# khanhha/temporal_inverse_kinematics

Hardware: AMD Instinct MI355X
Metric: IK frames/sec (COCO-17->SMPLx pose) (higher is better)
Workload: dtype f32 via bf16x3 (x = 3 bf16 planes, 6 MFMA products, fp32 accumulate; fp32 exponent range); 1 GPU; ST-GCN IK forward, batch=1024x64-frame x COCO-17 windows per GPU -> (B,4,66) SMPL-X pose; global_batch=1024, window_frames=64, out_frames=4, parallelism=single

## Files before the change

### temporal_inverse_kinematics_amd/csrc/xblock.hip

```cpp
#include <algorithm>
#include <type_traits>

#include "xgemm_dev.h"
#include "xblock.h"
#include "common.h"

namespace tik {

namespace xb {
constexpr int V = 17, C = 64, F = 10, FIN = F + 2;
constexpr int ROWB = 3 * C * 2;
constexpr int ZROWS = FIN * V;
constexpr int ZBYTES = (ZROWS + 1) * ROWB;
constexpr int XUNITS = ZROWS * 24, XINST = (XUNITS + 63) / 64;
constexpr int XBYTES = XINST * 1024;
constexpr int B2BYTES = V * C * 4;
constexpr int SMEM1 = ZBYTES + XBYTES + B2BYTES;
constexpr int F0 = 14, FIN0 = F0 + 2;
constexpr int ZBYTES0 = (FIN0 * V + 1) * ROWB;
constexpr int KPBYTES0 = FIN0 * V * 4 * 4;
constexpr int UBYTES0 = FIN0 * V * 16;
constexpr int SMEM0 = ZBYTES0 + KPBYTES0 + UBYTES0;
static_assert(SMEM1 <= 163840 && SMEM0 <= 163840, "LDS");
}

__device__ __forceinline__ int xb_unit(int R, int plane, int u) { return R * xb::ROWB + plane * 128 + ((u ^ (R & 7)) << 4); }
__device__ __forceinline__ int xb_xunit(int R, int j, int plane, int u) { return R * xb::ROWB + plane * 128 + ((u ^ ((R + j) & 7)) << 4); }

template <bool RAW>
__global__ __launch_bounds__(512, 1) void xblock_kernel(XBlkArgs a) {
    using namespace xb;
    constexpr int F = RAW ? F0 : xb::F, FIN = F + 2, ZROWS = FIN * V, ZR = ZROWS, ZBYTES = (ZROWS + 1) * ROWB;
    constexpr int KPBYTES = FIN * V * 4 * 4;
    constexpr int TPX = F * V, TBLK = (TPX + 15) / 16;
    static_assert(FIN <= 16, "one frame per lane of a 16-lane group");
    __shared__ __attribute__((aligned(16))) unsigned char smem[RAW ? SMEM0 : SMEM1];
    unsigned char* const zimg = smem;
    unsigned char* const ximg = smem + ZBYTES;
    float* const b2s = reinterpret_cast<float*>(smem + ZBYTES + XBYTES);

    int tid = threadIdx.x, lane = tid & 63;
    const int wave = __builtin_amdgcn_readfirstlane(tid >> 6);
    int g = lane >> 4;
    const int cg = wave & 3, ph = wave >> 2;
    const int QO = a.nframes, T = a.T;
    const int ntiles = (QO + F - 1) / F;
    int t_begin, t_end;
    {
        const int nwg = gridDim.x, bid = blockIdx.x;
        const int per = nwg >> 3, rem = nwg & 7, x = bid & 7, k = bid >> 3;
        const int s = x < rem ? x * (per + 1) + k : rem * (per + 1) + (x - rem) * per + k;
        t_begin = (int)((long long)s * ntiles / nwg);
        t_end = (int)((long long)(s + 1) * ntiles / nwg);
    }
    if (t_begin >= t_end) return;

    xbf16x8 wt[3][2][3];
    auto load_wt = [&]() __attribute__((always_inline)) {
        const unsigned short* wp = a.wtp;
        asm volatile("" : "+s"(wp));
#pragma unroll
        for (int k = 0; k < 3; ++k)
#pragma unroll
            for (int kb = 0; kb < 2; ++kb)
#pragma unroll
                for (int p = 0; p < 3; ++p)
                    wt[k][kb][p] = *reinterpret_cast<const xbf16x8*>(wp + ((((size_t)cg * 6 + k * 2 + kb) * 3 + p) * 64 + lane) * 8);
    };
    xbf16x8 wg[RAW ? 1 : 2][3];
    if constexpr (!RAW) {
#pragma unroll
        for (int kb = 0; kb < 2; ++kb)
#pragma unroll
            for (int p = 0; p < 3; ++p)
                wg[kb][p] = *reinterpret_cast<const xbf16x8*>(a.wgp + ((((size_t)cg * 2 + kb) * 3 + p) * 64 + lane) * 8);
    }
    float amv[5];
#pragma unroll
    for (int k = 0; k < 5; ++k) amv[k] = 64 * k + lane < V * V ? a.amix[64 * k + lane] : 0.f;
    int cho = 16 * cg + 4 * g;
    const f32x4 bv = *reinterpret_cast<const f32x4*>(a.bias + cho);
    float rw[4][4];
#pragma unroll
    for (int e = 0; e < 4; ++e)
#pragma unroll
        for (int c = 0; c < 4; ++c) rw[e][c] = RAW && c < a.c0 ? a.rw[(cho + e) * a.c0 + c] : 0.f;

    for (int i = tid; i < ROWB / 16; i += 512) *reinterpret_cast<f32x4*>(zimg + ZR * ROWB + 16 * i) = f32x4{0.f, 0.f, 0.f, 0.f};
    if constexpr (!RAW)
        for (int i = tid; i < V * C; i += 512) b2s[i] = a.bias2[i];

    const i32x4 rX = buf_rsrc(RAW ? nullptr : (const void*)a.xp3, RAW ? 0u : (unsigned)((long long)QO * V * ROWB));
    constexpr int NXI = (XINST + 7) / 8;
    unsigned xpre[NXI];
#pragma unroll
    for (int i = 0; i < NXI; ++i) {
        const int ins = wave + 8 * i;
        const int U = ins * 64 + lane;
        const int R = U / 24, k = U - R * 24, plane = k >> 3, up = k & 7;
        const int j = R / FIN, f = R - j * FIN;
        xpre[i] = U < XUNITS && ins < XINST ? (unsigned)((f * V + j) * ROWB + plane * 128 + ((up ^ ((R + j) & 7)) << 4)) | ((unsigned)f << 24)
                                            : 0x80000000u;
    }
    auto issue_x = [&](int tile) __attribute__((always_inline)) {
        const int q0 = tile * F;
#pragma unroll
        for (int i = 0; i < NXI; ++i) {
            const int ins = wave + 8 * i;
            if (ins >= XINST) break;
            const unsigned c = xpre[i];
            const int q = q0 - 1 + (int)((c >> 24) & 0x7F);
            const bool ok = !(c >> 31) && q >= 0 && q < QO;
            const unsigned off = ok ? (unsigned)((long long)(q0 - 1) * V * ROWB) + (c & 0xFFFFFFu) : DMA_OOB;
            tik_llvm_raw_buffer_load_lds(rX, (__attribute__((address_space(3))) unsigned*)(ximg + ins * 1024), 16, (int)off, 0, 0, 2);
        }
    };
    constexpr int KNE = RAW ? (FIN * V * 4 + 511) / 512 : 1;
    float kx[KNE], ksc[KNE], ksh[KNE];
    bool kok[KNE];
    auto load_kp = [&](int tile) __attribute__((always_inline)) {
#pragma unroll
        for (int jj = 0; jj < KNE; ++jj) {
            const int i = tid + 512 * jj, c = i & 3, p = i >> 2;
            const int v = p % V, fr = tile * F - 1 + p / V;
            kok[jj] = RAW && i < FIN * V * 4 && c < a.c0 && fr >= 0 && fr < QO;
            kx[jj] = kok[jj] ? a.xraw[((size_t)fr * V + v) * a.c0 + c] : 0.f;
        }
    };
    if constexpr (RAW) {
#pragma unroll
        for (int jj = 0; jj < KNE; ++jj) {
            const int i = tid + 512 * jj, c = i & 3, v = (i >> 2) % V;
            const bool ok = i < FIN * V * 4 && c < a.c0;
            ksc[jj] = ok ? a.bn_sc[v * a.c0 + c] : 0.f;
            ksh[jj] = ok ? a.bn_sh[v * a.c0 + c] : 0.f;
        }
        load_kp(t_begin);
    } else {
        asm volatile("s_waitcnt lgkmcnt(0)" ::: "memory");
        issue_x(t_begin);
    }

    constexpr int NB = (TBLK + 1) / 2;
    const int blk0 = ph * NB;
    const int nblk = ph == 0 ? NB : TBLK - NB;

#ifdef TIK_XTRACE
    const bool tr = a.trace != nullptr && (wave == 0 || wave == 4);
#else
    constexpr bool tr = false;
#endif
    unsigned long long ph_[8] = {0, 0, 0, 0, 0, 0, 0, 0}, tlast = 0;
    auto stamp = [&](int i) __attribute__((always_inline)) {
        if (tr) {
            const unsigned long long t = __builtin_amdgcn_s_memtime();
            if (i >= 0) ph_[i] += t - tlast;
            tlast = t;
        }
    };
    load_wt();
#pragma unroll
    for (int k = 0; k < 3; ++k)
#pragma unroll
        for (int kb = 0; kb < 2; ++kb)
#pragma unroll
            for (int p = 0; p < 3; ++p) asm volatile("" : "+v"(wt[k][kb][p]));
    for (int tile = t_begin; tile < t_end; ++tile) {
        const int q0 = tile * F;
        stamp(-1);
        asm volatile("" : "+v"(tid), "+v"(lane));
        g = lane >> 4;
        cho = 16 * cg + 4 * g;
        if constexpr (RAW) {
            float* kps = reinterpret_cast<float*>(ximg);
#pragma unroll
            for (int jj = 0; jj < KNE; ++jj) {
                const int i = tid + 512 * jj;
                if (i < FIN * V * 4) kps[i] = kok[jj] ? fmaf(kx[jj], ksc[jj], ksh[jj]) : 0.f;
            }
            __syncthreads();
            stamp(0);
            if (tile + 1 < t_end) load_kp(tile + 1);
            f32x4* const us = reinterpret_cast<f32x4*>(ximg + KPBYTES);
            {
                const int fl = lane;
                if (fl < FIN) {
#pragma unroll
                    for (int wj = 0; wj < V; ++wj)
                        if ((wj & 7) == wave) {
                            if (a.mix_sparse) us[fl * V + wj] = l0_mix_in<true>(kps + fl * V * 4, amv, wj);
                            else us[fl * V + wj] = l0_mix_in<false>(kps + fl * V * 4, amv, wj);
                        }
                }
            }
            __syncthreads();
            const int f = tid & 15, c4 = (tid >> 4) & 15, half = wave >> 2, co = 4 * c4;
            if (f < FIN) {
                float w[4][4];
#pragma unroll
                for (int e = 0; e < 4; ++e)
#pragma unroll
                    for (int c = 0; c < 4; ++c) w[e][c] = c < a.c0 ? a.wg0[(co + e) * a.ldwg0 + c] : 0.f;
                auto conv_half = [&](auto w0c, auto w1c) __attribute__((always_inline)) {
                    constexpr int W0 = decltype(w0c)::value, W1 = decltype(w1c)::value;
#pragma unroll
                    for (int wj = W0; wj < W1; ++wj) {
                        const f32x4 z = l0_conv_relu(us[f * V + wj], w, *reinterpret_cast<const f32x4*>(a.bias2 + wj * C + co));
                        xbf16x8 p0, p1, p2;
                        xsplit8(z, z, p0, p1, p2);
                        const int R = f * V + wj, u = co >> 3, o = (co & 7) * 2;
                        typedef __bf16 xbf16x4 __attribute__((ext_vector_type(4)));
                        *reinterpret_cast<xbf16x4*>(zimg + xb_unit(R, 0, u) + o) = xbf16x4{p0[0], p0[1], p0[2], p0[3]};
                        *reinterpret_cast<xbf16x4*>(zimg + xb_unit(R, 1, u) + o) = xbf16x4{p1[0], p1[1], p1[2], p1[3]};
                        *reinterpret_cast<xbf16x4*>(zimg + xb_unit(R, 2, u) + o) = xbf16x4{p2[0], p2[1], p2[2], p2[3]};
                    }
                };
                using I0 = std::integral_constant<int, 0>;
                using I9 = std::integral_constant<int, 9>;
                using I17 = std::integral_constant<int, 17>;
                if (half) conv_half(I9{}, I17{});
                else conv_half(I0{}, I9{});
            }
        } else {
            asm volatile("s_waitcnt vmcnt(0)" ::: "memory");
            __syncthreads();
            stamp(0);
            auto run_half = [&](auto jhc) __attribute__((always_inline)) {
                constexpr int JH = decltype(jhc)::value, J0 = JH ? 9 : 0, J1 = JH ? V : 9;
                f32x4 acc[V];
#pragma unroll
                for (int j = 0; j < V; ++j) acc[j] = f32x4{0.f, 0.f, 0.f, 0.f};
                const int fs = lane & 15, fr = fs < FIN ? fs : fs - FIN;
                constexpr int XPF = 2, S0 = 2 * J0, S1 = 2 * J1;
                xbf16x8 xb[XPF + 1][3];
                auto rd = [&](int s, xbf16x8 (&d)[3]) __attribute__((always_inline)) {
                    const int R = (s >> 1) * FIN + fr, kb = s & 1;
#pragma unroll
                    for (int p = 0; p < 3; ++p) d[p] = *reinterpret_cast<const xbf16x8*>(ximg + xb_xunit(R, s >> 1, p, 4 * kb + g));
                };
#pragma unroll
                for (int s = S0; s < S0 + XPF; ++s) rd(s, xb[(s - S0) % (XPF + 1)]);
#pragma unroll
                for (int s = S0; s < S1; ++s) {
                    const int j = s >> 1, kb = s & 1;
                    if (s + XPF < S1) rd(s + XPF, xb[(s + XPF - S0) % (XPF + 1)]);
                    __builtin_amdgcn_sched_barrier(0);
                    const xbf16x8(&x)[3] = xb[(s - S0) % (XPF + 1)];
                    acc[j] = __builtin_amdgcn_mfma_f32_16x16x32_bf16(wg[kb][0], x[2], acc[j], 0, 0, 0);
                    acc[j] = __builtin_amdgcn_mfma_f32_16x16x32_bf16(wg[kb][1], x[1], acc[j], 0, 0, 0);
                    acc[j] = __builtin_amdgcn_mfma_f32_16x16x32_bf16(wg[kb][2], x[0], acc[j], 0, 0, 0);
                    acc[j] = __builtin_amdgcn_mfma_f32_16x16x32_bf16(wg[kb][0], x[1], acc[j], 0, 0, 0);
                    acc[j] = __builtin_amdgcn_mfma_f32_16x16x32_bf16(wg[kb][1], x[0], acc[j], 0, 0, 0);
                    acc[j] = __builtin_amdgcn_mfma_f32_16x16x32_bf16(wg[kb][0], x[0], acc[j], 0, 0, 0);
                    __builtin_amdgcn_sched_barrier(0);
                }
                f32x4* xch = reinterpret_cast<f32x4*>(zimg);
#pragma unroll
                for (int j = J0; j < J1; ++j) xch[(j * 4 + cg) * 64 + lane] = acc[j];
                asm volatile("s_waitcnt lgkmcnt(0)" ::: "memory");
                __builtin_amdgcn_s_barrier();
#pragma unroll
                for (int j = 0; j < V; ++j)
                    if (j < J0 || j >= J1) acc[j] = xch[(j * 4 + cg) * 64 + lane];
                asm volatile("s_waitcnt lgkmcnt(0)" ::: "memory");
                __builtin_amdgcn_s_barrier();
                if (fs < FIN) {
                    auto mix_half = [&](auto sparse) __attribute__((always_inline)) {
                        constexpr bool SP = decltype(sparse)::value;
#pragma unroll
                        for (int w = J0; w < J1; ++w) {
                            f32x4 z = *reinterpret_cast<const f32x4*>(b2s + w * C + cho);
#pragma unroll
                            for (int v = 0; v < V; ++v)
                                if (!SP || ((coco_hop2_mask3(w) >> v) & 1u)) {
                                    const float av = __builtin_bit_cast(
                                        float, __builtin_amdgcn_readlane(__builtin_bit_cast(int, amv[(v * V + w) / 64]), (v * V + w) % 64));
                                    z += av * acc[v];
                                }
#pragma unroll
                            for (int e = 0; e < 4; ++e) z[e] = z[e] > 0.f ? z[e] : 0.f;
                            xbf16x8 p0, p1, p2;
                            xsplit8(z, z, p0, p1, p2);
                            const int R = fs * V + w, u = cho >> 3, o = (cho & 7) * 2;
                            typedef __bf16 xbf16x4 __attribute__((ext_vector_type(4)));
                            *reinterpret_cast<xbf16x4*>(zimg + xb_unit(R, 0, u) + o) = xbf16x4{p0[0], p0[1], p0[2], p0[3]};
                            *reinterpret_cast<xbf16x4*>(zimg + xb_unit(R, 1, u) + o) = xbf16x4{p1[0], p1[1], p1[2], p1[3]};
                            *reinterpret_cast<xbf16x4*>(zimg + xb_unit(R, 2, u) + o) = xbf16x4{p2[0], p2[1], p2[2], p2[3]};
                        }
                    };
                    if (a.mix_sparse) mix_half(std::true_type{});
                    else mix_half(std::false_type{});
                }
            };
            if (ph == 0) run_half(std::integral_constant<int, 0>{});
            else run_half(std::integral_constant<int, 1>{});
        }
        stamp(1);
        __syncthreads();
        stamp(2);

        f32x4 res[NB];
#pragma unroll
        for (int b = 0; b < NB; ++b) {
            const int p = (blk0 + b) * 16 + (lane & 15);
            const int fo = p / V, jt = p - fo * V;
            res[b] = f32x4{0.f, 0.f, 0.f, 0.f};
            if (b < nblk && p < TPX) {
                if constexpr (RAW) {
                    const float* xp = reinterpret_cast<const float*>(ximg) + ((fo + 1) * V + jt) * 4;
                    res[b] = f32x4{xp[0], xp[1], xp[2], xp[3]};
                } else {
                    const int R = jt * FIN + fo + 1, u = cho >> 3, o = (cho & 7) * 2;
                    typedef __bf16 xbf16x4 __attribute__((ext_vector_type(4)));
                    const xbf16x4 h0 = *reinterpret_cast<const xbf16x4*>(ximg + xb_xunit(R, jt, 0, u) + o);
                    const xbf16x4 h1 = *reinterpret_cast<const xbf16x4*>(ximg + xb_xunit(R, jt, 1, u) + o);
                    const xbf16x4 h2 = *reinterpret_cast<const xbf16x4*>(ximg + xb_xunit(R, jt, 2, u) + o);
#pragma unroll
                    for (int e = 0; e < 4; ++e) res[b][e] = ((float)h0[e] + (float)h1[e]) + (float)h2[e];
                }
            }
        }
        if constexpr (!RAW) {
            stamp(6);
            lds_barrier();
            if (tile + 1 < t_end) issue_x(tile + 1);
            stamp(7);
        }
        stamp(3);

        int rows[NB][3];
#pragma unroll
        for (int b = 0; b < NB; ++b) {
            const int p = (blk0 + b) * 16 + (lane & 15);
            const int fo = p / V, jt = p - fo * V;
            const int q = q0 + fo, tw = q % T;
#pragma unroll
            for (int k = 0; k < 3; ++k) {
                const bool ok = b < nblk && p < TPX && q < QO && tw + k - 1 >= 0 && tw + k - 1 < T;
                rows[b][k] = ok ? (fo + k) * V + jt : ZR;
            }
        }
        {
            constexpr int ZPF = 2, NS = 6 * NB;
            xbf16x8 zb[ZPF + 1][3];
            auto rdz = [&](int i, xbf16x8 (&d)[3]) __attribute__((always_inline)) {
                const int b = i / 6, s = i % 6, k = s % 3, kb = s / 3;
#pragma unroll
                for (int pl = 0; pl < 3; ++pl) d[pl] = *reinterpret_cast<const xbf16x8*>(zimg + xb_unit(rows[b][k], pl, 4 * kb + g));
            };
#pragma unroll
            for (int i = 0; i < ZPF; ++i) rdz(i, zb[i]);
            f32x4 acc = f32x4{0.f, 0.f, 0.f, 0.f};
#pragma unroll
            for (int i = 0; i < NS; ++i) {
                const int b = i / 6, s = i % 6;
                if (b >= nblk) break;
                if (i + ZPF < NS) rdz(i + ZPF, zb[(i + ZPF) % (ZPF + 1)]);
                __builtin_amdgcn_sched_barrier(0);
                const xbf16x8(&z)[3] = zb[i % (ZPF + 1)];
                const xbf16x8(&w)[3] = wt[s % 3][s / 3];
                acc = __builtin_amdgcn_mfma_f32_16x16x32_bf16(w[0], z[2], acc, 0, 0, 0);
                acc = __builtin_amdgcn_mfma_f32_16x16x32_bf16(w[1], z[1], acc, 0, 0, 0);
                acc = __builtin_amdgcn_mfma_f32_16x16x32_bf16(w[2], z[0], acc, 0, 0, 0);
                acc = __builtin_amdgcn_mfma_f32_16x16x32_bf16(w[0], z[1], acc, 0, 0, 0);
                acc = __builtin_amdgcn_mfma_f32_16x16x32_bf16(w[1], z[0], acc, 0, 0, 0);
                acc = __builtin_amdgcn_mfma_f32_16x16x32_bf16(w[0], z[0], acc, 0, 0, 0);
                __builtin_amdgcn_sched_barrier(0);
                if (s < 5) continue;
                const int p = (blk0 + b) * 16 + (lane & 15);
                const int fo = p / V;
                const int q = q0 + fo;
                const long long row = (long long)q0 * V + p;
                const bool st = p < TPX && q < QO;
                f32x4 v = acc;
                acc = f32x4{0.f, 0.f, 0.f, 0.f};
                if constexpr (RAW) {
                    v += bv;
#pragma unroll
                    for (int e = 0; e < 4; ++e) {
                        v[e] += res[b][0] * rw[e][0] + res[b][1] * rw[e][1] + res[b][2] * rw[e][2] + res[b][3] * rw[e][3];
                        v[e] = v[e] > 0.f ? v[e] : 0.f;
                    }
                    xbf16x8 p0, p1, p2;
                    xsplit8(v, v, p0, p1, p2);
                    typedef __bf16 xbf16x4 __attribute__((ext_vector_type(4)));
                    unsigned short* o = st ? a.out_p3 + row * (3 * C) + cho : reinterpret_cast<unsigned short*>(a.trash);
                    *reinterpret_cast<xbf16x4*>(o) = xbf16x4{p0[0], p0[1], p0[2], p0[3]};
                    *reinterpret_cast<xbf16x4*>(o + C) = xbf16x4{p1[0], p1[1], p1[2], p1[3]};
                    *reinterpret_cast<xbf16x4*>(o + 2 * C) = xbf16x4{p2[0], p2[1], p2[2], p2[3]};
                } else {
                    v += res[b];
                    v += bv;
#pragma unroll
                    for (int e = 0; e < 4; ++e) v[e] = v[e] > 0.f ? v[e] : 0.f;
                    float* o = st ? a.out_f + row * C + cho : a.trash;
                    *reinterpret_cast<f32x4*>(o) = v;
                }
            }
        }
        asm volatile("s_waitcnt lgkmcnt(0)" ::: "memory");
        stamp(4);
        __syncthreads();
        stamp(5);
    }
    if (tr && lane == 0) {
        unsigned long long* o = a.trace + 24 * (size_t)blockIdx.x + (wave == 4 ? 12 : 0);
        for (int i = 0; i < 8; ++i) o[i] = ph_[i];
        o[8] = t_end - t_begin; o[9] = 1;
    }
    asm volatile("s_waitcnt vmcnt(0)" ::: "memory");
}

hipError_t launch_xblock(const XBlkArgs& a, bool raw, int ncu, hipStream_t st) {
    if (a.nframes <= 0) return hipSuccess;
    if (a.T <= 0 || !a.wtp || !a.amix || !a.bias || !a.trash || ncu <= 0) return hipErrorInvalidValue;
    if (raw && (!a.xraw || a.c0 < 1 || a.c0 > 4 || !a.bn_sc || !a.bn_sh || !a.wg0 || a.ldwg0 < a.c0 || !a.rw || !a.out_p3 || !a.bias2))
        return hipErrorInvalidValue;
    if (!raw && (!a.xp3 || !a.wgp || !a.bias2 || !a.out_f)) return hipErrorInvalidValue;
    if (!raw && (long long)a.nframes * xb::V * xb::ROWB >= (1LL << 31)) return hipErrorInvalidValue;
    const int f = raw ? xb::F0 : xb::F;
    const int ntiles = (a.nframes + f - 1) / f;
    const int grid = std::min(ntiles, ncu);
    (void)hipGetLastError();
    if (raw) hipLaunchKernelGGL(xblock_kernel<true>, dim3(grid), dim3(512), 0, st, a);
    else hipLaunchKernelGGL(xblock_kernel<false>, dim3(grid), dim3(512), 0, st, a);
    return hipGetLastError();
}

int xblock_frames_per_tile() { return xb::F; }
int xblock0_frames_per_tile() { return xb::F0; }

std::vector<unsigned short> xblock_pack_weights(const float* w, int cout, int ldw, int kt, int cin) {
    const int nkb = cin / 32, ns = kt * nkb, ncg = cout / 16;
    std::vector<unsigned short> out((size_t)ncg * ns * 3 * 64 * 8, 0);
    for (int c = 0; c < ncg; ++c)
        for (int tap = 0; tap < kt; ++tap)
            for (int kb = 0; kb < nkb; ++kb)
                for (int l = 0; l < 64; ++l)
                    for (int e = 0; e < 8; ++e) {
                        const int co = 16 * c + (l & 15), ci = 32 * kb + 8 * (l >> 4) + e;
                        unsigned short p[3];
                        tik_host::split_bf16x3(w[(size_t)co * ldw + (size_t)tap * cin + ci], p[0], p[1], p[2]);
                        const int s = tap * nkb + kb;
                        for (int pl = 0; pl < 3; ++pl) out[((((size_t)c * ns + s) * 3 + pl) * 64 + l) * 8 + e] = p[pl];
                    }
    return out;
}

}
```

Measured before the change: 337,400 IK frames/s.

## Interleave next-tile X DMA into the MFMA loop and drop a per-tile barrier

Splits the next-tile X prefetch into individual buffer-to-LDS loads. They are issued one every T_DMA_STEP MFMA steps inside the temporal-conv loop, instead of as a burst after an LDS barrier. The residual reads and row/boundary precomputation move ahead of a single __syncthreads, using wave ballots for window-edge detection. The end-of-tile __syncthreads is removed. The aim is to spread DMA issue across compute and cut barrier stalls per tile, at the risk of LDS hazards when the next tile's X overwrites data still being read.

```diff
diff --git a/temporal_inverse_kinematics_amd/csrc/xblock.hip b/temporal_inverse_kinematics_amd/csrc/xblock.hip
--- a/temporal_inverse_kinematics_amd/csrc/xblock.hip
+++ b/temporal_inverse_kinematics_amd/csrc/xblock.hip
@@ -22,6 +22,7 @@
 constexpr int UBYTES0 = FIN0 * V * 16;
 constexpr int SMEM0 = ZBYTES0 + KPBYTES0 + UBYTES0;
 static_assert(SMEM1 <= 163840 && SMEM0 <= 163840, "LDS");
+constexpr int T_DMA_STEP = 2;
 }
 
 __device__ __forceinline__ int xb_unit(int R, int plane, int u) { return R * xb::ROWB + plane * 128 + ((u ^ (R & 7)) << 4); }
@@ -102,18 +103,20 @@
         xpre[i] = U < XUNITS && ins < XINST ? (unsigned)((f * V + j) * ROWB + plane * 128 + ((up ^ ((R + j) & 7)) << 4)) | ((unsigned)f << 24)
                                             : 0x80000000u;
     }
+    auto issue_x1 = [&](int tile, int i) __attribute__((always_inline)) {
+        const int q0 = tile * F;
+        const unsigned base = (unsigned)(q0 - 1) * (unsigned)(V * ROWB);
+        const int ins = wave + 8 * i;
+        if (ins >= XINST) return;
+        const unsigned c = xpre[i];
+        const int q = q0 - 1 + (int)((c >> 24) & 0x7F);
+        const bool ok = !(c >> 31) && q >= 0 && q < QO;
+        const unsigned off = ok ? base + (c & 0xFFFFFFu) : DMA_OOB;
+        tik_llvm_raw_buffer_load_lds(rX, (__attribute__((address_space(3))) unsigned*)(ximg + ins * 1024), 16, (int)off, 0, 0, 2);
+    };
     auto issue_x = [&](int tile) __attribute__((always_inline)) {
-        const int q0 = tile * F;
-#pragma unroll
-        for (int i = 0; i < NXI; ++i) {
-            const int ins = wave + 8 * i;
-            if (ins >= XINST) break;
-            const unsigned c = xpre[i];
-            const int q = q0 - 1 + (int)((c >> 24) & 0x7F);
-            const bool ok = !(c >> 31) && q >= 0 && q < QO;
-            const unsigned off = ok ? (unsigned)((long long)(q0 - 1) * V * ROWB) + (c & 0xFFFFFFu) : DMA_OOB;
-            tik_llvm_raw_buffer_load_lds(rX, (__attribute__((address_space(3))) unsigned*)(ximg + ins * 1024), 16, (int)off, 0, 0, 2);
-        }
+#pragma unroll
+        for (int i = 0; i < NXI; ++i) issue_x1(tile, i);
     };
     constexpr int KNE = RAW ? (FIN * V * 4 + 511) / 512 : 1;
     float kx[KNE], ksc[KNE], ksh[KNE];
@@ -296,50 +299,43 @@
             else run_half(std::integral_constant<int, 1>{});
         }
         stamp(1);
-        __syncthreads();
-        stamp(2);
-
+
+        static_assert(F <= 16, "one output frame per lane of a 16-lane group");
+        const int twl = (q0 + (lane & 15)) % T;
+        const unsigned wfirst = (unsigned)__ballot(twl == 0), wlast = (unsigned)__ballot(twl == T - 1);
+        int rows[NB][3];
         f32x4 res[NB];
+        unsigned stm = 0;
 #pragma unroll
         for (int b = 0; b < NB; ++b) {
             const int p = (blk0 + b) * 16 + (lane & 15);
             const int fo = p / V, jt = p - fo * V;
-            res[b] = f32x4{0.f, 0.f, 0.f, 0.f};
-            if (b < nblk && p < TPX) {
-                if constexpr (RAW) {
-                    const float* xp = reinterpret_cast<const float*>(ximg) + ((fo + 1) * V + jt) * 4;
-                    res[b] = f32x4{xp[0], xp[1], xp[2], xp[3]};
-                } else {
-                    const int R = jt * FIN + fo + 1, u = cho >> 3, o = (cho & 7) * 2;
-                    typedef __bf16 xbf16x4 __attribute__((ext_vector_type(4)));
-                    const xbf16x4 h0 = *reinterpret_cast<const xbf16x4*>(ximg + xb_xunit(R, jt, 0, u) + o);
-                    const xbf16x4 h1 = *reinterpret_cast<const xbf16x4*>(ximg + xb_xunit(R, jt, 1, u) + o);
-                    const xbf16x4 h2 = *reinterpret_cast<const xbf16x4*>(ximg + xb_xunit(R, jt, 2, u) + o);
-#pragma unroll
-                    for (int e = 0; e < 4; ++e) res[b][e] = ((float)h0[e] + (float)h1[e]) + (float)h2[e];
-                }
+            const bool live = b < nblk && p < TPX, inq = live && q0 + fo < QO;
+            if (p < TPX && q0 + fo < QO) stm |= 1u << b;
+            rows[b][0] = inq && !((wfirst >> fo) & 1u) ? p : ZR;
+            rows[b][1] = inq ? p + V : ZR;
+            rows[b][2] = inq && !((wlast >> fo) & 1u) ? p + 2 * V : ZR;
+            if constexpr (RAW) {
+                const f32x4 kp = *reinterpret_cast<const f32x4*>(ximg + (live ? p + V : 0) * 16);
+                res[b] = live ? kp : f32x4{0.f, 0.f, 0.f, 0.f};
+            } else {
+                const int R = live ? jt * FIN + fo + 1 : 0, js = live ? jt : 0, u = cho >> 3, o = (cho & 7) * 2;
+                typedef __bf16 xbf16x4 __attribute__((ext_vector_type(4)));
+                const xbf16x4 h0 = *reinterpret_cast<const xbf16x4*>(ximg + xb_xunit(R, js, 0, u) + o);
+                const xbf16x4 h1 = *reinterpret_cast<const xbf16x4*>(ximg + xb_xunit(R, js, 1, u) + o);
+                const xbf16x4 h2 = *reinterpret_cast<const xbf16x4*>(ximg + xb_xunit(R, js, 2, u) + o);
+#pragma unroll
+                for (int e = 0; e < 4; ++e) res[b][e] = live ? ((float)h0[e] + (float)h1[e]) + (float)h2[e] : 0.f;
             }
         }
-        if constexpr (!RAW) {
-            stamp(6);
-            lds_barrier();
-            if (tile + 1 < t_end) issue_x(tile + 1);
-            stamp(7);
-        }
+        stamp(6);
+        __syncthreads();
+        stamp(2);
+        constexpr int XDS = T_DMA_STEP;
+        static_assert(RAW || (NXI - 1) * XDS < 6 * (TBLK - NB), "every DMA inside the shorter half's T");
+        [[maybe_unused]] const bool xnext = tile + 1 < t_end;
         stamp(3);
 
-        int rows[NB][3];
-#pragma unroll
-        for (int b = 0; b < NB; ++b) {
-            const int p = (blk0 + b) * 16 + (lane & 15);
-            const int fo = p / V, jt = p - fo * V;
-            const int q = q0 + fo, tw = q % T;
-#pragma unroll
-            for (int k = 0; k < 3; ++k) {
-                const bool ok = b < nblk && p < TPX && q < QO && tw + k - 1 >= 0 && tw + k - 1 < T;
-                rows[b][k] = ok ? (fo + k) * V + jt : ZR;
-            }
-        }
         {
             constexpr int ZPF = 2, NS = 6 * NB;
             xbf16x8 zb[ZPF + 1][3];
@@ -355,6 +351,8 @@
             for (int i = 0; i < NS; ++i) {
                 const int b = i / 6, s = i % 6;
                 if (b >= nblk) break;
+                if constexpr (!RAW)
+                    if (i % XDS == 0 && i / XDS < NXI && xnext) issue_x1(tile + 1, i / XDS);
                 if (i + ZPF < NS) rdz(i + ZPF, zb[(i + ZPF) % (ZPF + 1)]);
                 __builtin_amdgcn_sched_barrier(0);
                 const xbf16x8(&z)[3] = zb[i % (ZPF + 1)];
@@ -368,10 +366,8 @@
                 __builtin_amdgcn_sched_barrier(0);
                 if (s < 5) continue;
                 const int p = (blk0 + b) * 16 + (lane & 15);
-                const int fo = p / V;
-                const int q = q0 + fo;
                 const long long row = (long long)q0 * V + p;
-                const bool st = p < TPX && q < QO;
+                const bool st = (stm >> b) & 1u;
                 f32x4 v = acc;
                 acc = f32x4{0.f, 0.f, 0.f, 0.f};
                 if constexpr (RAW) {
@@ -400,7 +396,6 @@
         }
         asm volatile("s_waitcnt lgkmcnt(0)" ::: "memory");
         stamp(4);
-        __syncthreads();
         stamp(5);
     }
     if (tr && lane == 0) {
```

Result: no change. 339,700 IK frames/s (median of 6 runs) (+0.7%).
